# kai422/DAS3R

Hardware: AMD Instinct MI355X
Metric: render fwd+bwd Msplats/s at 1080p (higher is better)
Workload: dtype f32; 1 GPU; 1M random splats, 1920x1080, SH degree 3, forward+backward (BASELINE.json configs[3], constant P); splats_per_gpu=1000000, splats_per_gpu_final=1000000, init_steps=30, sh_degree=3, num_rendered=2614506, api=GaussianRasterizer.forward + autograd backward (drop-in surface), parallelism=1 independent scenes, one per GPU

## Files before the change

### das3r_amd/csrc/api.hip

```cpp
#include <stdarg.h>
#include <string.h>

#include <vector>

#include "common.h"
#include <algorithm>

namespace das3r {

static thread_local char g_err[512] = "";

void set_error(const char *fmt, ...) {
    va_list ap;
    va_start(ap, fmt);
    vsnprintf(g_err, sizeof(g_err), fmt, ap);
    va_end(ap);
}

struct ProfRec {
    const char *name;
    hipEvent_t start, stop;
};
static bool g_prof_on = false;
static std::vector<ProfRec> g_prof;
bool profile_enabled() { return g_prof_on; }
static std::vector<hipEvent_t> g_event_pool;
static hipEvent_t pooled_event() {
    if (!g_event_pool.empty()) { hipEvent_t e = g_event_pool.back(); g_event_pool.pop_back(); return e; }
    hipEvent_t e = nullptr;
    return hipEventCreate(&e) == hipSuccess ? e : nullptr;
}
void profile_begin(const char *name, hipStream_t s) {
    ProfRec r;
    r.name = name;
    r.start = pooled_event();
    r.stop = pooled_event();
    if (!r.start || !r.stop) return;
    (void)hipEventRecord(r.start, s);
    g_prof.push_back(r);
}
void profile_end(hipStream_t s) {
    if (!g_prof.empty()) (void)hipEventRecord(g_prof.back().stop, s);
}

static Switches g_sw;
static bool g_sw_loaded = false;
static int g_inject_fault = 0;
static int g_mutate = 0;
static void load_switches() {
    Switches w;
    memset(&w, 0, sizeof(w));
    auto env = [](const char *k) -> const char * { const char *e = getenv(k); return (e && e[0]) ? e : nullptr; };
    const char *e;
#ifdef DAS3R_EXPERIMENTS
    if ((e = env("DAS3R_SORT_IPL"))) { const int v = atoi(e); w.sort_ipl = (v == 4 || v == 8 || v == 16) ? v : 0; }
    w.sort_classic = (e = env("DAS3R_SORT")) && e[0] == 'c';
    w.no_sh_stage = getenv("DAS3R_NO_SH_STAGE") != nullptr;
    if ((e = env("DAS3R_ABLATE"))) { w.ablate_set = true; w.ablate = atoi(e); }
    if ((e = env("DAS3R_BWD_PAD_LDS"))) w.bwd_pad_lds = atoi(e);
    if ((e = env("DAS3R_FWD_PAD_LDS"))) w.fwd_pad_lds = atoi(e);
    if ((e = env("DAS3R_SCAN_ITEMS"))) { const int v = atoi(e); w.scan_items = (v == 1 || v == 2 || v == 4 || v == 8 || v == 16) ? v : 0; }
    w.fwd_no_prefetch = (e = env("DAS3R_FWD_PREFETCH")) && e[0] == '0';
#endif
    w.rect_upstream = (e = env("DAS3R_RECT")) && e[0] == 'u';
    w.verbose = env("DAS3R_VERBOSE") != nullptr;
    if ((e = env("DAS3R_BINNING"))) w.binning = e[0] == 'l' ? 1 : (e[0] == 'r' ? -1 : (e[0] == 's' ? (strchr(e, '3') ? 3 : 2) : 0));
    w.capacity_exact = (e = env("DAS3R_CAPACITY")) && e[0] == 'e';
    w.fused_emit_off = (e = env("DAS3R_FUSED_EMIT")) && e[0] == '0';
    if ((e = env("DAS3R_SPLIT_COLOUR"))) w.split_colour = e[0] == '0' ? -1 : (e[0] == '1' ? 1 : 0);
    w.tile_lpt_off = (e = env("DAS3R_TILE_LPT")) && e[0] == '0';
    if ((e = env("DAS3R_RENDER"))) w.render_fwd = e[0] == 'q' ? 1 : (e[0] == 'r' ? 2 : (e[0] == 'l' ? 3 : (e[0] == 's' ? 4 : (e[0] == 'f' ? 5 : 0))));
    if ((e = env("DAS3R_RENDER_BWD"))) {
        w.render_bwd = e[0] == 'd' ? 1 : (e[0] == 'm' ? 2 : (strncmp(e, "stream", 6) == 0 ? 5 : (e[0] == 's' ? 3 : (e[0] == 'b' ? 6 : (e[0] == 'f' ? 7 : 0)))));
        if (w.render_bwd == 6) {
            const char *d = e;
            while (*d && (*d < '0' || *d > '9')) d++;
            w.render_bwd_mb = *d ? atoi(d) : 128;
            const char *pp = strchr(e, 'p');
            w.render_bwd_pix = pp ? atoi(pp + 1) : 0;
            const char *po = strchr(e, 'o');
            w.render_bwd_occ = po ? atoi(po + 1) : 5;
        }
        if (w.render_bwd == 7) {
            const char *d = e;
            while (*d && (*d < '0' || *d > '9')) d++;
            w.render_bwd_mb = *d ? atoi(d) : 128;
            w.render_bwd_pix = strchr(e, 'q') ? 9 : (strchr(e, 's') ? 8 : 0);
        }
        if (w.render_bwd == 3) {
            const char *d = e;
            while (*d && (*d < '0' || *d > '9')) d++;
            w.render_bwd_mb = (*d ? atoi(d) : 256) + (strncmp(e, "scana", 5) == 0 ? 1000 : 0);
        }
    }
    if ((e = env("DAS3R_BWD_REDUCE"))) { w.bwd_reduce_set = true; w.bwd_reduce_shfl = e[0] == 's'; }
    w.tickets = -1;
    if ((e = env("DAS3R_TICKETS"))) w.tickets = e[0] == 'a' ? 0 : (e[0] == 'n' ? 1 << 30 : ((e[0] >= '1' && e[0] <= '9') ? atoi(e) : -1));
    w.deterministic = (e = env("DAS3R_DETERMINISTIC")) && e[0] != '0';
    w.bwd_buckets = -1;
    if ((e = env("DAS3R_BWD_BUCKETS"))) w.bwd_buckets = atoi(e);
    w.tile_strip = 8;
    w.tile_chunk = -1;
    if ((e = env("DAS3R_TILE_CHUNK"))) { const int v = atoi(e); w.tile_chunk = (v >= 0 && v <= 64 && (v & (v - 1)) == 0) ? v : -1; }
    if ((e = env("DAS3R_TILE_STRIP"))) w.tile_strip = std::max(0, std::min(63, atoi(e)));
    w.inject_fault = g_inject_fault;
    w.mutate = g_mutate;
    g_sw = w;
    __atomic_store_n(&g_sw_loaded, true, __ATOMIC_RELEASE);
}
const Switches &switches() {
    if (!__atomic_load_n(&g_sw_loaded, __ATOMIC_ACQUIRE)) load_switches();
    return g_sw;
}

constexpr int MAX_DEVICES = 64;
static int g_threads_on_device[MAX_DEVICES] = {};
struct ThreadRegistrar {
    bool on[MAX_DEVICES] = {};
    void add(int dev) {
        if (!on[dev]) { on[dev] = true; __atomic_fetch_add(&g_threads_on_device[dev], 1, __ATOMIC_RELAXED); }
    }
    ~ThreadRegistrar() {
// ... 31 lines not shown
    if (forced > 0) return true;
    return sh_degree >= 2 && P >= SPLIT_MIN_P && !no_backward;
}

struct SideStreams {
    struct Entry { int dev; hipStream_t caller; SideStream ss; };
    std::vector<Entry> all;
    ~SideStreams() {
        for (auto &e : all) {
            (void)hipEventDestroy(e.ss.fork);
            (void)hipEventDestroy(e.ss.join);
            (void)hipStreamDestroy(e.ss.stream);
        }
    }
};
static int side_stream_for(hipStream_t s, SideStream *out) {
    static thread_local SideStreams streams;
    int dev = 0;
    HIP_TRY(hipGetDevice(&dev));
    for (auto &e : streams.all)
        if (e.dev == dev && e.caller == s) { *out = e.ss; return DAS3R_OK; }
    SideStream ss = {nullptr, nullptr, nullptr, 0};
    int cus = 0;
    HIP_TRY(hipDeviceGetAttribute(&cus, hipDeviceAttributeMultiprocessorCount, dev));
    ss.colour_blocks = COLOUR_WGS_PER_CU * (cus > 0 ? cus : 1);
    HIP_TRY(hipStreamCreateWithFlags(&ss.stream, hipStreamNonBlocking));
    HIP_TRY(hipEventCreateWithFlags(&ss.fork, hipEventDisableTiming));
    HIP_TRY(hipEventCreateWithFlags(&ss.join, hipEventDisableTiming));
    streams.all.push_back(SideStreams::Entry{dev, s, ss});
    *out = ss;
    return DAS3R_OK;
}

int sort_ipl_override() { return switches().sort_ipl; }
#ifdef DAS3R_EXPERIMENTS
bool use_onesweep() { return !switches().sort_classic; }
#else
bool use_onesweep() { return true; }
#endif
bool use_tight_rect() { return !switches().rect_upstream; }

void compute_layout(int P, int64_t I, int W, int H, Layout *L, bool shjac) {
    memset(L, 0, sizeof(*L));
    const size_t Pn = P > 0 ? (size_t)P : 1, In = I > 0 ? (size_t)I : 1;
    L->capacity = I;
    L->tiles_x = (W + TILE_X - 1) / TILE_X;
    L->tiles_y = (H + TILE_Y - 1) / TILE_Y;
    L->ntiles = L->tiles_x * L->tiles_y;
    L->tbits = tile_bits(L->ntiles);
    L->tile_passes = (L->tbits + 7) / 8;
    L->dbits = 0;
    L->kbits = L->tbits;
    L->kshift = 0;
    L->part_passes = L->tile_passes;
    L->chunksP = sort_num_chunks(P);
    L->chunksI = sort_num_chunks(I);
    size_t o = 0;
    auto take = [&](size_t b) { size_t r = o; o += align_up(b); return r; };
    L->g_keyA = take(4 * Pn);
    L->g_keyB = take(4 * Pn);
    L->g_valA = take(4 * Pn);
    L->g_valB = take(4 * Pn);
    L->pub.sorted_idx = L->g_valA;
    L->pub.depth_key = L->g_keyA;
    L->pub.xy = take(16 * SPLAT_REC * Pn);
    L->pub.conic_opacity = L->pub.xy + 16;
    L->pub.rgbd = L->pub.xy + 32;
    L->pub.splat_stride = 16 * SPLAT_REC;
    L->pub.clamped = take(Pn);
    L->pub.tiles_touched = take(4 * Pn);
    L->pub.offsets = take(4 * Pn);
    L->g_hist = take(4 * (size_t)RADIX_SIZE * (size_t)(L->chunksP > 0 ? L->chunksP : 1));
    L->g_totals = take(4 * RADIX_SIZE);
    L->g_blocksums = take(4 * (size_t)div_up((int64_t)Pn, 4096));
    L->g_count = take(256);
    L->g_off_by_gid = take(4 * Pn);
    L->g_rect = take(4 * Pn);
    L->g_dhist = take(4 * 256);
    L->g_ghist = take(4 * 4 * RADIX_SIZE);
    L->g_ticket = take(256);
    L->g_status = take(onesweep_status_bytes((int64_t)Pn, 4));
    L->g_scan_status = take(scan_status_bytes((int)Pn));
    L->g_ctrl_bytes = o - L->g_ghist;
    if (shjac) L->g_shjac = take(4 * 9 * Pn);
    L->pub.geom_bytes = o;
    o = 0;
    L->b_keyA = take(4 * In);
    L->b_keyB = take(4 * In);
    L->b_valA = take(4 * In);
    L->b_valB = take(4 * In);
    L->b_hist = take(4 * (size_t)RADIX_SIZE * (size_t)(L->chunksI > 0 ? L->chunksI : 1));
    L->b_totals = take(4 * RADIX_SIZE);
    L->b_gid_of = take(4 * In);
    L->b_slot = take(4 * In);
    L->b_e2 = take(4 * In);
    L->b_ghist = take(4 * 4 * RADIX_SIZE);
    L->b_ticket = take(256);
    L->b_status = take(onesweep_status_bytes((int64_t)In, L->tile_passes + 1));
    L->b_ctrl_bytes = o - L->b_ghist;
    L->b_ckpt = take(((size_t)In / BUCKET + (size_t)(L->ntiles > 0 ? L->ntiles : 1) + 2) * 256 * 16);
    L->pub.binning_bytes = o;
    const size_t npix_d = (size_t)W * (size_t)H;
    L->d_ckpt = take(((size_t)In / BUCKET + (size_t)(L->ntiles > 0 ? L->ntiles : 1) + 2) * 256 * 16);
    L->d_recs = take(16 * SPLAT_REC * Pn);
    L->d_dpix = take(4 * 3 * (npix_d > 0 ? npix_d : 1));
    L->d_bg = take(16);
// ... 245 lines not shown
    Mailbox *mb = &T->mb;
    auto check_slot = [&](uint32_t i, bool wait) -> int {
        if (!T->pending[i]) return DAS3R_OK;
        const int r = examine_check_slot(mb->host + CHECK_WORD0 + 2 * i, T->pending[i], wait, s);
        if (r == 1) return DAS3R_OK;
        T->pending[i] = 0;
        return r;
    };
    for (uint32_t i = 0; i < CHECK_SLOTS; i++)
        if ((rc = check_slot(i, false))) return rc;
    uint32_t late_tag = 0;
    unsigned long long *&arrive_ring = T->arrive_ring;
    constexpr uint32_t ARRIVE_SLOTS = 16, ARRIVE_WORDS = 8 + 64 * 8;
    if (!arrive_ring) {
        HIP_TRY(hipMalloc((void **)&arrive_ring, ARRIVE_SLOTS * ARRIVE_WORDS * sizeof(unsigned long long)));
        HIP_TRY(hipMemsetAsync(arrive_ring, 0, ARRIVE_SLOTS * ARRIVE_WORDS * sizeof(unsigned long long), s));
        HIP_TRY(hipStreamSynchronize(s));
    }
    Verdict &verdict = T->verdict;
    constexpr int64_t LOCAL_AVG = 384;
    const uint32_t too_long = mb->host[10];
    if (too_long) mb->host[10] = 0;
    const uint32_t want_bits = mb->host[11];
    if (want_bits) mb->host[11] = 0;
    if (verdict.P != P || verdict.W != W || verdict.H != H) {
        const uint32_t gen = verdict.gen + 1u ? verdict.gen + 1u : 1u;
        verdict = Verdict{P, W, H, -1, 0, 0, 64, gen};
        if (T->pending_valid) {
            verdict.fine = T->pending_fine;
            verdict.forwards = T->pending_forwards;
            T->pending_valid = false;
        }
    }
    const bool decide_fine = (verdict.forwards++ & 511u) == 0u;
    auto next_gen = [&]() { verdict.gen = verdict.gen + 1u ? verdict.gen + 1u : 1u; };
    if (verdict.last_I < 0) {
    } else if (too_long == verdict.gen && !(verdict.last_seg && verdict.seg_extra == 0 && L.tile_passes < 3 && seg_dbits(L, L.tile_passes + 1) > 0)) {
        if (verdict.clean >= 256u) verdict.backoff = 64;
        verdict.radix_left = verdict.backoff;
        if (verdict.backoff < 4096) verdict.backoff *= 2;
        verdict.clean = 0;
        next_gen();
    } else if (too_long == verdict.gen || want_bits == verdict.gen) {
        verdict.seg_extra = 1;
        next_gen();
    }
    const int forced = switches().binning;
    bool local = use_onesweep() && (forced == 1 || (forced == 0 && verdict.radix_left == 0 && verdict.last_I <= LOCAL_AVG * L.ntiles));
    constexpr int64_t SEG_AVG = 384;
    const int seg_passes = L.tile_passes + ((forced == 3 || (forced == 0 && verdict.seg_extra)) ? 1 : 0);
    const int seg_bits = (use_onesweep() && seg_passes <= 3) ? seg_dbits(L, seg_passes) : 0;
    bool seg = !local && seg_bits > 0 && (forced >= 2 || (forced == 0 && verdict.radix_left == 0 && verdict.last_I >= 0 &&
                                                           (verdict.last_I >> std::min(seg_bits, 20)) <= SEG_AVG * L.ntiles));
    const uint32_t *seg_dhist = nullptr;
    auto apply_seg = [&]() {
        L.dhist_ptr = seg_dhist;
        if (seg) {
            L.dbits = seg_bits;
            L.kbits = L.tbits + seg_bits;
            L.kshift = std::min(16, 32 - L.kbits);
            L.part_passes = seg_passes;
        }
    };
    verdict.last_seg = seg;
    if (local || seg) verdict.clean++;
    if (forced == 0 && verdict.radix_left > 0) verdict.radix_left--;
    const uint32_t count_tag = ++mb->seq ? mb->seq : ++mb->seq;
    unsigned long long *arrive = arrive_ring + (size_t)(count_tag % ARRIVE_SLOTS) * ARRIVE_WORDS;
    struct Join {
        hipStream_t s;
        const das3r_raster_args *a;
        const das3r_raster_in *in;
        char *const *geom;
        const Layout *L;
        SideStream side;
        bool forked, pending;
        int launch() {
            if (!forked) return DAS3R_OK;
            forked = false;
            pending = true;
            return launch_sh_colour(a, in, *geom, *L, &side);
        }
        int now() {
            const int r = launch();
            if (r) return r;
            if (!pending) return DAS3R_OK;
            pending = false;
            HIP_TRY(hipStreamWaitEvent(s, side.join, 0));
            return DAS3R_OK;
        }
        ~Join() {
            if (pending) (void)hipStreamWaitEvent(s, side.join, 0);
        }
    } join = {s, a, in, &saved->geom, &L, {nullptr, nullptr, nullptr, 0}, false, false};
    auto split_side = [&](int binning_path, const SideStream **side) -> int {
        *side = nullptr;
        if (!split_colour_rule(in->shs != nullptr, a->sh_degree, P, binning_path, no_backward, switches().split_colour)) return DAS3R_OK;
        const int r = side_stream_for(s, &join.side);
        if (r) return r;
        *side = &join.side;
        return DAS3R_OK;
    };
    auto bin_and_render = [&](int64_t cap, bool local_order, bool ctrl_zeroed, uint32_t *count_out = nullptr, uint32_t count_out_tag = 0,
                              uint32_t *emit_slot = nullptr ) -> int {
        int r;
        const bool fused_scan = use_onesweep();
        const bool seg = L.dbits > 0;
        if (!emit_slot) {
            if (fused_scan) {
                if ((r = launch_binning_scan_emit(P, cap, out->radii, saved->geom, saved->binning, L, ctrl_zeroed, count_out, count_out_tag, a->debug != 0,
                                                  s, local_order || seg))) return r;
            } else if ((r = launch_scan(P, saved->geom, L, nullptr, 0, a->debug != 0, s))) return r;
        }
        uint32_t *host_late = nullptr;
        if (cap > 0) {
            late_tag = ++mb->seq ? mb->seq : ++mb->seq;
            const uint32_t slot = late_tag % CHECK_SLOTS;
            if ((r = check_slot(slot, true))) return r;
            T->pending[slot] = late_tag;
            host_late = mb->dev + CHECK_WORD0 + 2 * slot;
            saved->check_word = (void *)(mb->host + CHECK_WORD0 + 2 * slot);
            saved->check_tag = late_tag;
        }
        uint32_t *dead_keys = nullptr;
        if ((r = launch_binning(P, cap, W, H, out->radii, saved->geom, saved->binning, saved->img, L, fused_scan, host_late, late_tag,
                                a->debug != 0, s, &dead_keys, emit_slot, mb->dev + 10, verdict.gen))) return r;
        if ((r = join.launch())) return r;
        LocalBin lb = {(float4 *)(saved->binning + L.b_ckpt), nullptr, nullptr, nullptr, nullptr, verdict.gen, (uint32_t)(P - 1), (uint32_t)cap};
        if (decide_fine && cap > 0 && use_quad_lanes(L, lb)) {
            const uint32_t tag = ++mb->seq ? mb->seq : ++mb->seq;
            if ((r = launch_list_skew(saved->img, saved->binning, saved->geom, L, (uint32_t)cap, (uint32_t)(P - 1), mb->dev + 13, tag, a->debug != 0, s))) return r;
            if ((r = mailbox_wait(mb, 14, tag, s))) return r;
            const int64_t longest = (int64_t)mb->host[13], mean = (verdict.last_I > 0 ? verdict.last_I : cap) / std::max(L.ntiles, 1);
            verdict.longest = (uint32_t)longest;
            const uint32_t crowd16 = mb->host[15];
            verdict.fine = (longest > mean + (mean * 4) / 5 && longest >= 4096) || crowd16 >= CROWDED16;
            if (switches().verbose) fprintf(stderr, "[das3r] tile lists: longest %lld, mean %lld, %.1f of 64 consecutive entries in one quadrant -> %s kernels\n", (long long)longest,
                                            (long long)mean, crowd16 / 16.0, verdict.fine ? "2x2-region" : "block");
        }
        lb.prefer_regions = verdict.fine;
        lb.tile_order = nullptr;
        if (verdict.fine && cap > 0 && use_quad_lanes(L, lb) && L.ntiles <= 1024 && !switches().tile_lpt_off && (switches().render_fwd == 0 || switches().render_fwd == 5)) {
            if ((r = launch_tile_lpt(saved->img, L, (uint32_t)cap, a->debug != 0, s))) return r;
            lb.tile_order = (const uint32_t *)(saved->img + L.i_order);
        }
        if (verdict.fine && cap > 0 && use_quad_lanes(L, lb)) {
            const uint32_t hint = std::min<uint32_t>(63u, verdict.longest / (uint32_t)BUCKET + 2u);
            saved->flags |= 1u | (hint << 8);
        }
        if (local_order && cap > 0) {
            lb.point_list = (uint32_t *)(saved->binning + L.pub.point_list);
            lb.slot_list = (uint32_t *)(saved->binning + L.b_slot);
            lb.keys = dead_keys;
            lb.host_flag = mb->dev + 10;
        }
        if ((r = join.now())) return r;
        return launch_render_forward(a, in->colors_precomp, out->out_color, saved->geom, saved->binning, saved->img, L, lb, s, out->out_invdepth,
                                     depth ? (float4 *)(saved->binning + L.d_ckpt) : nullptr);
    };
    auto prefiltered_ok = [&]() -> int {
        if (!a->prefiltered || mb->host[12] != count_tag) return DAS3R_OK;
        set_error("Point is filtered although prefiltered is set. This shouldn't happen!");
        return DAS3R_ERR_INVALID_ARG;
    };
    int64_t I, cap;
    if ((local || seg) && verdict.last_I >= 0 && a->capacity_hint != -1 && !switches().capacity_exact) {
        cap = std::max(verdict.last_I + verdict.last_I / 4, verdict.peak_I + verdict.peak_I / 20) + 4096;
        if (cap > (int64_t)0x7FFFFF00) cap = (int64_t)0x7FFFFF00;
        compute_layout(P, cap, W, H, &L, shjac);
        apply_seg();
        saved->binning = alloc_binning(user, depth ? L.d_bytes : L.pub.binning_bytes);
        if (!saved->binning) { set_error("scratch allocation failed (binning %zu B)", L.pub.binning_bytes); return DAS3R_ERR_ALLOC; }
        char *&emit_ring = T->emit_ring;
        bool &emit_ring_dirty = T->emit_ring_dirty;
        uint32_t &emit_last_tag = T->emit_last_tag;
        constexpr size_t EMIT_SLOT_BYTES = sizeof(uint32_t) * EMIT_SLOT_WORDS + sizeof(unsigned long long) * EMIT_STATUS_GRANULES;
        const bool fused_emit = local && grid_is_resident(div_up(P, 256)) && !switches().fused_emit_off;
        uint32_t *emit_slot = nullptr;
        if (fused_emit) {
            if (!emit_ring) {
                HIP_TRY(hipMalloc((void **)&emit_ring, ARRIVE_SLOTS * EMIT_SLOT_BYTES));
                emit_ring_dirty = true;
            }
            if (emit_ring_dirty || count_tag < emit_last_tag) {
                HIP_TRY(hipMemsetAsync(emit_ring, 0, ARRIVE_SLOTS * EMIT_SLOT_BYTES, s));
                emit_ring_dirty = false;
            }
            emit_last_tag = count_tag;
            emit_slot = (uint32_t *)(emit_ring + (size_t)(count_tag % ARRIVE_SLOTS) * EMIT_SLOT_BYTES);
            const EmitArgs em = {(unsigned long long *)(emit_slot + EMIT_SLOT_WORDS), count_tag, emit_slot + 64, emit_slot,
                                 (uint32_t *)(saved->binning + L.b_keyA), (uint32_t *)(saved->binning + L.b_gid_of),
                                 (uint32_t *)(saved->geom + L.g_off_by_gid), (uint32_t)cap, L.tbits, (uint32_t *)(saved->geom + L.g_count), mb->dev};
            emit_ring_dirty = true;
            if ((rc = launch_preprocess(a, in, out->radii, saved->geom, saved->img, saved->binning + L.b_ghist, L.b_ctrl_bytes, L, nullptr, mb->dev,
                                        count_tag, s, &em, nullptr, nullptr, aa))) return rc;
            if ((rc = bin_and_render(cap, true, true, nullptr, 0, emit_slot))) return rc;
            emit_ring_dirty = false;
        } else {
            uint32_t *dhist = nullptr, *dhist_next = nullptr;
            if (seg && !dhist_slots(s, &dhist, &dhist_next)) {
                dhist = (uint32_t *)(saved->geom + L.g_dhist);
                HIP_TRY(hipMemsetAsync(dhist, 0, 4 * 256, s));
            }
            seg_dhist = dhist;
            apply_seg();
            const SideStream *side = nullptr;
            if ((rc = split_side(1, &side))) return rc;
            if ((rc = launch_preprocess(a, in, out->radii, saved->geom, saved->img, saved->binning + L.b_ghist, L.b_ctrl_bytes, L, nullptr, mb->dev,
                                        count_tag, s, nullptr, dhist, dhist_next, aa, side))) return rc;
            join.forked = side != nullptr;
            if ((rc = bin_and_render(cap, local, true, mb->dev, count_tag))) return rc;
        }
        if ((rc = mailbox_wait(mb, 2, count_tag, s))) return rc;
        if ((rc = prefiltered_ok())) return rc;
        I = (int64_t)mb->host[0];
        if (I > (int64_t)0x7FFFFF00) { set_error("num_rendered %lld exceeds 2^31", (long long)I); return DAS3R_ERR_OVERFLOW; }
        verdict.last_I = I;
        verdict.peak_I = std::max(I, verdict.peak_I - verdict.peak_I / 1024);
        if (I > cap) {
            cap = I;
            compute_layout(P, cap, W, H, &L, shjac);
            saved->binning = alloc_binning(user, depth ? L.d_bytes : L.pub.binning_bytes);
            if (!saved->binning) { set_error("scratch allocation failed (binning %zu B)", L.pub.binning_bytes); return DAS3R_ERR_ALLOC; }
            apply_seg();
            HIP_TRY(hipMemsetAsync(saved->geom + L.g_ghist, 0, L.g_ctrl_bytes, s));
            HIP_TRY(hipMemsetAsync(saved->img + L.pub.ranges, 0, 8 * (size_t)L.ntiles, s));
            if ((rc = bin_and_render(cap, local, false))) return rc;
        }
    } else {
        uint32_t *dhist = nullptr, *dhist_next = nullptr;
        if (seg && !dhist_slots(s, &dhist, &dhist_next)) {
            dhist = (uint32_t *)(saved->geom + L.g_dhist);
            HIP_TRY(hipMemsetAsync(dhist, 0, 4 * 256, s));
        }
        seg_dhist = dhist;
        const SideStream *side = nullptr;
        if ((rc = split_side((local || seg) ? 1 : 0, &side))) return rc;
        if ((rc = launch_preprocess(a, in, out->radii, saved->geom, saved->img, nullptr, 0, L, arrive, mb->dev, count_tag, s, nullptr, dhist, dhist_next, aa, side))) return rc;
        join.forked = side != nullptr;
        if (!local && !seg && (rc = launch_depth_sort(P, saved->geom, L, 0, nullptr, 0, a->debug != 0, s))) return rc;
        if ((rc = mailbox_wait(mb, 2, count_tag, s))) return rc;
        if ((rc = prefiltered_ok())) return rc;
        I = cap = (int64_t)mb->host[0];
        if (cap > (int64_t)0x7FFFFF00) { set_error("num_rendered %lld exceeds 2^31", (long long)cap); return DAS3R_ERR_OVERFLOW; }
        verdict.last_I = I;
        verdict.peak_I = std::max(I, verdict.peak_I - verdict.peak_I / 1024);
        if (local && forced == 0 && I > LOCAL_AVG * L.ntiles) {
            local = false;
            if ((rc = join.now())) return rc;
            if ((rc = launch_depth_sort(P, saved->geom, L, 0, nullptr, 0, a->debug != 0, s))) return rc;
        }
        compute_layout(P, cap, W, H, &L, shjac);
        apply_seg();
        saved->binning = alloc_binning(user, depth ? L.d_bytes : L.pub.binning_bytes);
        if (!saved->binning) { set_error("scratch allocation failed (binning %zu B)", L.pub.binning_bytes); return DAS3R_ERR_ALLOC; }
        if (!local && !seg && (rc = launch_depth_sort(P, saved->geom, L, 1, saved->binning + L.b_ghist, L.b_ctrl_bytes, a->debug != 0, s))) return rc;
        if ((rc = bin_and_render(cap, local, !local && !seg))) return rc;
    }
    if (a->debug && late_tag && (rc = check_slot(late_tag % CHECK_SLOTS, true))) return rc;
    saved->num_rendered = I;
    saved->capacity = cap;
    if (depth) saved->flags |= DEPTH_SAVED_FLAG;
    if (shjac) saved->flags |= SHJAC_SAVED_FLAG;
    return I;
}

static bool shjac_saved(const das3r_raster_args *a, const das3r_raster_in *in, const das3r_raster_saved *saved) {
    return (saved->flags & SHJAC_SAVED_FLAG) != 0 && in->shs != nullptr && a->sh_degree >= 2;
}

extern "C" int das3r_raster_backward(const das3r_raster_args *a, const das3r_raster_in *in, const das3r_raster_saved *saved,
                                     const float *dL_dpix, const das3r_raster_grads *g, das3r_stream_t stream) {
    hipStream_t s = (hipStream_t)stream;
    int rc = validate(a, in);
    if (rc) return rc;
    const int P = a->P;
    if (P == 0) return DAS3R_OK;
    const bool chained = g && g->chain;
    if (!saved || !saved->geom || !saved->img || !dL_dpix || !g || !g->dL_dmeans2D || (!chained && (!g->dL_dopacities || !g->dL_dmeans3D)) ||
        (saved && saved->num_rendered > 0 && !g->scratch)) {
        set_error("das3r_raster_backward: null saved state / gradient buffer");
        return DAS3R_ERR_INVALID_ARG;
    }
    const bool has_sh = in->shs != nullptr, has_cov = in->cov3D_precomp != nullptr;
// ... 280 lines not shown
```

### das3r_amd/csrc/common.h

```cpp
#pragma once
#include <hip/hip_runtime.h>
#include <stdint.h>
#include <stdio.h>

#include "../../include/das3r_raster.h"
#include "pretransform_math.h"

#define TILE_X 16
#define TILE_Y 16
#define TILE_PIX 256
#define WAVE 64
#define NEAR_PLANE 0.001f

namespace das3r {

void set_error(const char *fmt, ...);

struct Switches {
    int sort_ipl;
    bool sort_classic;
    bool rect_upstream;
    bool verbose;
    int binning;
    bool capacity_exact;
    bool fused_emit_off;
    bool no_sh_stage;
    int render_fwd;
    int render_bwd;
    int render_bwd_mb;
    int tile_chunk;
    int scan_items;
    bool deterministic;
    int render_bwd_occ;
    bool tile_lpt_off;
    int render_bwd_pix;
    bool bwd_reduce_set, bwd_reduce_shfl;
    bool ablate_set;
    int ablate;
    int tickets;
    int bwd_pad_lds, fwd_pad_lds;
    int bwd_buckets;
    int inject_fault;
    int mutate;
    bool fwd_no_prefetch;
    int split_colour;
    int tile_strip;
};
const Switches &switches();

#define HIP_TRY(expr)                                                                          \
    do {                                                                                       \
        hipError_t _e = (expr);                                                                \
        if (_e != hipSuccess) {                                                                \
            das3r::set_error("%s failed: %s (%s:%d)", #expr, hipGetErrorString(_e), __FILE__, __LINE__); \
            return DAS3R_ERR_HIP;                                                              \
        }                                                                                      \
    } while (0)

#define KERNEL_CHECK(stream, debug, name)                                                      \
    do {                                                                                       \
        hipError_t _e = hipGetLastError();                                                     \
        if (_e == hipSuccess && (debug)) _e = hipStreamSynchronize(stream);                    \
        if (_e != hipSuccess) {                                                                \
            das3r::set_error("kernel %s failed: %s", name, hipGetErrorString(_e));             \
            return DAS3R_ERR_HIP;                                                              \
        }                                                                                      \
    } while (0)

bool profile_enabled();
void profile_begin(const char *name, hipStream_t s);
void profile_end(hipStream_t s);
struct ProfTimer {
    hipStream_t s;
    bool on;
    ProfTimer(const char *name, hipStream_t stream) : s(stream), on(profile_enabled()) {
        if (on) profile_begin(name, s);
    }
    ~ProfTimer() {
        if (on) profile_end(s);
    }
};

unsigned long long *pair_counters();
constexpr int PHASE_WORDS = 16, PHASE_COPIES = 64;
#ifdef DAS3R_EXPERIMENTS
#define PHASE_BEGIN()                                                                      \
    __shared__ unsigned long long phase_w_[8];                                             \
    unsigned long long phase_t_ = 0ull;                                                    \
    if (pairs != nullptr && threadIdx.x == 0) {                                            \
        for (int k_ = 0; k_ < 8; k_++) phase_w_[k_] = 0ull;                                \
        phase_t_ = clock64();                                                              \
    }
#define PHASE_MARK(k)                                                                      \
    if (pairs != nullptr && threadIdx.x == 0) {                                            \
        const unsigned long long now_ = clock64();                                         \
        phase_w_[(k) & 7] += now_ - phase_t_;                                              \
        phase_t_ = now_;                                                                   \
    }
// ... 30 lines not shown
#define WG_STAMP(k)
#define SCAN_STAMP(k)
#define BLK_STAMP(ptr, r, k)
#endif

#define DAS3R_LAUNCH(kernel, grid, block, shmem, stream, ...)                \
    do {                                                                     \
        das3r::ProfTimer _pt(#kernel, stream);                               \
        hipLaunchKernelGGL(kernel, grid, block, shmem, stream, __VA_ARGS__); \
    } while (0)

static inline size_t align_up(size_t x, size_t a = 256) { return (x + a - 1) / a * a; }
static inline int div_up(int64_t a, int64_t b) { return (int)((a + b - 1) / b); }

constexpr int RADIX_BITS = 8;
constexpr int RADIX_SIZE = 1 << RADIX_BITS;
constexpr int SORT_WAVES_PER_BLOCK = 4;
int sort_ipl_override();
static inline int sort_items_per_lane(int64_t n) {
    const int o = sort_ipl_override();
    return o ? o : (n >= (int64_t)(1 << 21) ? 16 : (n >= (1 << 17) ? 8 : 4));
}
static inline int sort_num_chunks(int64_t n) { return n == 0 ? 0 : div_up(n, (int64_t)WAVE * sort_items_per_lane(n)); }
__host__ __device__ static inline int tile_digit_width(int tbits) {
    const int passes = (tbits + 7) / 8;
    return passes > 0 ? (tbits + passes - 1) / passes : 8;
}
static inline int tile_bits(int ntiles) {
    int b = 0;
    while ((1 << b) < ntiles) b++;
    return b < 1 ? 1 : b;
}

constexpr int BUCKET = 1024;
constexpr int SPLAT_REC = 4;

constexpr uint32_t DEPTH_SAVED_FLAG = 2u;
constexpr uint32_t SHJAC_SAVED_FLAG = 4u;
constexpr uint32_t NO_BACKWARD_IN_FLAG = 8u;
constexpr uint32_t ANTIALIAS_FLAG = 16u;
struct Layout {
    das3r_raster_layout pub;
    size_t g_keyA, g_keyB, g_valA, g_valB, g_hist, g_totals, g_blocksums, g_count, g_off_by_gid, g_rect;
    size_t b_keyA, b_keyB, b_valA, b_valB, b_hist, b_totals, b_gid_of, b_slot;
    size_t b_e2;
    size_t b_ckpt;
    size_t d_ckpt, d_recs, d_dpix, d_bg, d_dz, d_bytes;
    size_t g_ghist, g_ticket, g_status, g_scan_status, g_ctrl_bytes;
    int64_t capacity;
    size_t b_ghist, b_ticket, b_status, b_ctrl_bytes;
    int tiles_x, tiles_y, ntiles, tbits, tile_passes;
    int chunksP, chunksI;
    int dbits, kbits, kshift;
    int part_passes;
    size_t g_dhist;
    size_t g_shjac;
    const uint32_t *dhist_ptr;
    size_t i_order;
};
static inline int seg_dbits(const Layout &L, int passes) { return 8 * (passes < 3 ? passes : 3) - L.tbits; }

struct LocalBin {
    float4 *ckpt;
    uint32_t *point_list, *slot_list;
    uint32_t *keys;
    uint32_t *host_flag;
    uint32_t flag_value;
    uint32_t last_g, cap;
    bool prefer_regions;
    const uint32_t *tile_order;
};
void compute_layout(int P, int64_t I, int W, int H, Layout *L, bool shjac = false);

struct EmitArgs {
    unsigned long long *status;
    uint32_t tag;
    uint32_t *ghist;
    uint32_t *err;
    uint32_t *tile_keys, *gids, *off_by_gid;
    uint32_t cap;
    int tbits;
    uint32_t *count;
    uint32_t *count_out;
};
constexpr int EMIT_SLOT_WORDS = 64 + 4 * 256;
constexpr int EMIT_STATUS_GRANULES = 1024;

constexpr int COLOUR_WGS_PER_CU = 4;
struct SideStream {
    hipStream_t stream;
    hipEvent_t fork, join;
    int colour_blocks;
};
int launch_preprocess(const das3r_raster_args *a, const das3r_raster_in *in, int32_t *radii, char *geom, char *img, char *binning_ctrl,
                      size_t binning_ctrl_bytes, const Layout &L, unsigned long long *arrive, uint32_t *host_out, uint32_t tag,
                      hipStream_t s, const EmitArgs *emit, uint32_t *dhist, uint32_t *dhist_next, bool aa ,
                      const SideStream *side = nullptr);
int launch_sh_colour(const das3r_raster_args *a, const das3r_raster_in *in, char *geom, const Layout &L, const SideStream *side);
int launch_mark_visible(int P, const float *means3D, const float *viewmatrix, uint8_t *present, hipStream_t s);
int launch_depth_sort(int P, char *geom, const Layout &L, int part, char *binning_ctrl, size_t binning_ctrl_bytes, bool debug, hipStream_t s);
int launch_scan(int P, char *geom, const Layout &L, uint32_t *host_out, uint32_t tag, bool debug, hipStream_t s, bool index_order = false);
int launch_scan_emit(int P, int64_t cap, const int32_t *radii, char *geom, char *binning, const Layout &L, uint32_t *host_out, uint32_t tag,
                     bool debug, hipStream_t s, bool index_order = false);
size_t scan_status_bytes(int P);
int launch_binning_scan_emit(int P, int64_t I, const int32_t *radii, char *geom, char *binning, const Layout &L, bool ctrl_zeroed,
                             uint32_t *host_out, uint32_t tag, bool debug, hipStream_t s, bool index_order = false);
size_t onesweep_status_bytes(int64_t n, int passes);
int launch_onesweep_depth_sort(int P, char *geom, const Layout &L, int part, uint32_t *zero_ptr, uint32_t zero_words, bool debug,
                               hipStream_t s);
int launch_onesweep_partition(int64_t cap, char *geom, char *binning, const Layout &L, uint32_t **keys_final, bool debug, hipStream_t s,
                              uint32_t *ghist_override = nullptr, uint32_t *err_override = nullptr);
bool use_row_private(int64_t instances, int ntiles);
bool use_quad_lanes(const Layout &L, const LocalBin &lb);
inline PreXform pre_xform(const das3r_raster_in *in) {
    PreXform x = {nullptr, nullptr, nullptr, nullptr, nullptr, nullptr, nullptr, nullptr, nullptr};
    if (in && in->pre) {
        const das3r_pretransform *p = in->pre;
        x = PreXform{p->xyz, p->rot, p->scaling, p->opacity_raw, p->conf_flat, p->mask_index, p->R, p->t, p->Lq};
    }
    return x;
}
int launch_render_forward_regions(const das3r_raster_args *a, float *out_color, char *geom, char *binning, char *img, const Layout &L, const LocalBin &lb,
                                  hipStream_t s, float *out_invdepth, float4 *dckpt);
// ... 80 lines not shown
```

### das3r_amd/csrc/render_common.h

```cpp
#pragma once
#include "common.h"

namespace das3r {

struct StagedSplat {
    float4 xyh;
    float4 co;
    float4 rgbd;
};

__device__ __forceinline__ float4 lds_read4(const float4 *p) {
    const float4 v = *p;
    asm volatile("" ::"v"(v.w));
    return v;
}

__device__ __forceinline__ StagedSplat null_splat() {
    StagedSplat z;
    z.xyh = make_float4(0.f, 0.f, -1e30f, -1e30f);
    z.co = make_float4(0.f, 0.f, 0.f, 0.f);
    z.rgbd = make_float4(0.f, 0.f, 0.f, 0.f);
    return z;
}

// ... 182 lines not shown
        for (int lk = 1; lk <= G; lk++) {
#pragma unroll
            for (int i = 0; i < E; i++)
                if (!(i & (1 << (lk - 1)))) ce64(v[i], v[i ^ ((1 << lk) - 1)]);
#pragma unroll
            for (int lj = lk - 2; lj >= 0; lj--)
#pragma unroll
                for (int i = 0; i < E; i++)
                    if (!((i >> lj) & 1)) ce64(v[i], v[i | (1 << lj)]);
        }
#pragma unroll
        for (int m = 0; m < E; m++) key[lane * E + m] = v[m];
    }
    __builtin_amdgcn_fence(__ATOMIC_ACQ_REL, "wavefront");
    for (int lk = G + 1; lk <= LOGN; lk++) {
        {
            const int sh = lk - G;
            const int block = lane >> sh, hbase = lane & ((1 << sh) - 1);
            const int lo0 = (block << lk) + hbase, hi0 = (block << lk) + ((1 << lk) - 1) - hbase;
            double a[H], b[H];
#pragma unroll
            for (int m = 0; m < H; m++) {
                a[m] = key[lo0 + (m << sh)];
                b[m] = key[hi0 - (m << sh)];
            }
#pragma unroll
            for (int m = 0; m < H; m++) ce64(a[m], b[m]);
#pragma unroll
            for (int t = G - 2; t >= 0; t--)
#pragma unroll
                for (int m = 0; m < H; m++)
                    if (!((m >> t) & 1)) {
                        ce64(a[m], a[m | (1 << t)]);
                        ce64(b[m | (1 << t)], b[m]);
                    }
#pragma unroll
            for (int m = 0; m < H; m++) {
                key[lo0 + (m << sh)] = a[m];
                key[hi0 - (m << sh)] = b[m];
            }
        }
        __builtin_amdgcn_fence(__ATOMIC_ACQ_REL, "wavefront");
        for (int R = lk - G; R > 0;) {
            const int g = R < G ? R : G;
            if (g == 1) butterfly_group<1, E>(key, lane, R);
            else if (g == 2) butterfly_group<2, E>(key, lane, R);
            else if (g == 3) butterfly_group<3, E>(key, lane, R);
            __builtin_amdgcn_fence(__ATOMIC_ACQ_REL, "wavefront");
            R -= g;
        }
    }
}

struct NoMark {
    __device__ __forceinline__ void operator()(int) const {}
};
template <bool DEPTH = false, class Mark = NoMark>
__device__ __forceinline__ bool local_order_tile(const LocalBin &lb, const uint2 range, const float4 *__restrict__ xyh,
                                                 const float4 *__restrict__ conic_opacity, const float4 *__restrict__ rgbd,
                                                 StagedSplat *stage , uint32_t *s_gid , const int tid,
                                                 const Mark mark = Mark()) {
    const int n = (int)(range.y - range.x);
    uint32_t *pl = lb.point_list + range.x, *sl = lb.slot_list + range.x;
    if (n <= TILE_PIX) {
        unsigned long long *s_key = reinterpret_cast<unsigned long long *>(s_gid);
        unsigned long long key = 0;
        uint32_t g = 0, slot = 0;
        float4 r0 = make_float4(0.f, 0.f, 0.f, 0.f), r1 = r0, r2 = r0;
        if (tid < n) {
            g = min(pl[tid], lb.last_g);
            slot = sl[tid];
            r0 = xyh[(size_t)g * SPLAT_REC];
            r1 = conic_opacity[(size_t)g * SPLAT_REC];
            r2 = rgbd[(size_t)g * SPLAT_REC];
            key = ((unsigned long long)__float_as_uint(r2.w) << 32) | (unsigned long long)g;
        }
        if (tid < ((n + 7) & ~7)) s_key[tid] = tid < n ? key : ~0ull;
        __syncthreads();
        if (tid < n) {
            int rank = 0;
            for (int j = 0; j < n; j += 8) {
                unsigned long long o[8];
#pragma unroll
                for (int u = 0; u < 8; u++) o[u] = s_key[j + u];
#pragma unroll
                for (int u = 0; u < 8; u++) rank += o[u] < key ? 1 : 0;
            }
            stage[rank].xyh = r0;
            stage[rank].co = r1;
            if constexpr (DEPTH) stage[rank].rgbd = staged_invz(r2);
            else stage[rank].rgbd = r2;
            pl[rank] = g;
            sl[rank] = slot;
        } else {
            stage[tid] = null_splat();
        }
        return true;
    }
    if (n <= LOCAL_MAX) {
        unsigned long long *s_key = reinterpret_cast<unsigned long long *>(stage);
        uint32_t *s_slot = reinterpret_cast<uint32_t *>(stage) + 2 * LOCAL_MAX;
        const int N = n <= 2 * TILE_PIX ? 2 * TILE_PIX : LOCAL_MAX;
        for (int i = tid; i < N; i += TILE_PIX) {
            unsigned long long k = SORT_PAD;
            if (i < n) {
                const uint32_t g = min(pl[i], lb.last_g);
                s_gid[i] = g;
                s_slot[i] = sl[i];
                k = ((unsigned long long)__float_as_uint(rgbd[(size_t)g * SPLAT_REC].w) << 32) | (unsigned long long)i;
            }
            s_key[i] = k;
        }
        __syncthreads();
        mark(6);
        if (N == 2 * TILE_PIX) {
            if (tid < 64) wave_bitonic_sort<3>(reinterpret_cast<double *>(stage), tid);
// ... 156 lines not shown
```

### das3r_amd/csrc/sort.hip

```cpp
#include "granule.h"
#include "segkey.h"
#include <algorithm>
#include "splat_math.h"

namespace das3r {

template <int IPL>
__global__ void __launch_bounds__(256) radix_hist_kernel(const uint32_t *__restrict__ keys, uint32_t cap, const uint32_t *__restrict__ n_ptr,
                                                         int shift, uint32_t mask, int nchunks, uint32_t *__restrict__ hist) {
    const uint32_t n = n_ptr ? min(*n_ptr, cap) : cap;
    __shared__ uint32_t cnt[SORT_WAVES_PER_BLOCK][RADIX_SIZE];
    const int lane = __lane_id(), wave = threadIdx.x >> 6;
    const int chunk = blockIdx.x * SORT_WAVES_PER_BLOCK + wave;
    const uint32_t base = (uint32_t)chunk * 64u * (uint32_t)IPL;
    uint32_t k[IPL];
#pragma unroll
    for (int s = 0; s < IPL; s++) {
        const uint32_t i = base + s * 64 + lane;
        k[s] = (chunk < nchunks && i < n) ? keys[i] : 0u;
    }
#pragma unroll
    for (int d = lane; d < RADIX_SIZE; d += 64) cnt[wave][d] = 0;
    __builtin_amdgcn_wave_barrier();
    if (chunk >= nchunks) return;
// ... 228 lines not shown
    uint32_t *hist = (uint32_t *)(geom + L.g_hist), *totals = (uint32_t *)(geom + L.g_totals);
    if (P == 0) return DAS3R_OK;
    int rc;
    if (use_onesweep()) return launch_onesweep_depth_sort(P, geom, L, part, (uint32_t *)binning_ctrl, (uint32_t)(binning_ctrl_bytes / 4), debug, s);
#ifdef DAS3R_EXPERIMENTS
    if (part == 1) return DAS3R_OK;
    if ((rc = radix_pass(keyA, nullptr, keyB, valB, P, 0, 8, hist, totals, debug, s))) return rc;
    if ((rc = radix_pass(keyB, valB, keyA, valA, P, 8, 8, hist, totals, debug, s))) return rc;
    if ((rc = radix_pass(keyA, valA, keyB, valB, P, 16, 8, hist, totals, debug, s))) return rc;
    if ((rc = radix_pass(keyB, valB, nullptr, valA, P, 24, 8, hist, totals, debug, s))) return rc;
#else
    (void)keyA; (void)keyB; (void)valA; (void)valB; (void)hist; (void)totals; (void)rc;
#endif
    return DAS3R_OK;
}

int launch_binning_scan_emit(int P, int64_t I, const int32_t *radii, char *geom, char *binning, const Layout &L, bool ctrl_zeroed,
                             uint32_t *host_out, uint32_t tag, bool debug, hipStream_t s, bool index_order) {
    if (I == 0 || P == 0) return DAS3R_OK;
    if (!ctrl_zeroed) HIP_TRY(hipMemsetAsync(binning + L.b_ghist, 0, L.b_ctrl_bytes, s));
    return launch_scan_emit(P, I, radii, geom, binning, L, host_out, tag, debug, s, index_order);
}

int launch_binning(int P, int64_t I, int W, int H, const int32_t *radii, char *geom, char *binning, char *img, const Layout &L,
                   bool fused_scan, uint32_t *host_late, uint32_t tag, bool debug, hipStream_t s, uint32_t **dead_keys, uint32_t *emit_slot,
                   uint32_t *seg_host_flag, uint32_t seg_flag_value) {
    const uint32_t *n_ptr = (const uint32_t *)(geom + L.g_count);
    (void)W; (void)H;
    uint2 *ranges = (uint2 *)(img + L.pub.ranges);
    if (I == 0 || P == 0) return DAS3R_OK;
    uint32_t *keyA = (uint32_t *)(binning + L.b_keyA), *keyB = (uint32_t *)(binning + L.b_keyB);
    uint32_t *valA = (uint32_t *)(binning + L.b_valA), *valB = (uint32_t *)(binning + L.b_valB);
    uint32_t *hist = (uint32_t *)(binning + L.b_hist), *totals = (uint32_t *)(binning + L.b_totals);
    uint32_t *gid_of = (uint32_t *)(binning + L.b_gid_of), *inv = (uint32_t *)(binning + L.b_slot);
    const bool onesweep = use_onesweep();
    (void)onesweep;
#ifdef DAS3R_EXPERIMENTS
    if (!fused_scan) {
    const int emit_blocks = div_up(P, 256) < 1024 ? div_up(P, 256) : 1024;
    DAS3R_LAUNCH(emit_kernel, dim3(emit_blocks), dim3(256), 0, s, P, L.tiles_x, L.tiles_y,
                 (const uint32_t *)(geom + L.pub.sorted_idx), (const uint32_t *)(geom + L.pub.tiles_touched),
                 (const uint32_t *)(geom + L.pub.offsets), (const float4 *)(geom + L.pub.xy), radii, keyA, gid_of, (uint32_t)I,
                 onesweep ? (uint32_t *)(binning + L.b_ghist) : (uint32_t *)nullptr, L.tbits, use_tight_rect() ? 1 : 0);
    KERNEL_CHECK(s, debug, "emit");
    }
#else
    (void)radii; (void)fused_scan; (void)gid_of;
#endif
    if (onesweep) {
        uint32_t *kfinal = nullptr;
        int rc1 = launch_onesweep_partition(I, geom, binning, L, &kfinal, debug, s, emit_slot ? emit_slot + 64 : nullptr, emit_slot);
        if (rc1) return rc1;
        if (dead_keys) *dead_keys = kfinal;
        if (L.dbits > 0) {
            uint32_t *other = kfinal == keyA ? keyB : keyA;
            return launch_segment_sort(I, n_ptr, kfinal, L.kshift, (uint32_t *)(binning + L.pub.point_list), (uint32_t *)(binning + L.b_slot),
                                       (const uint32_t *)(geom + L.pub.depth_key), (uint32_t)(P - 1), other, seg_host_flag, seg_flag_value, debug, s,
                                       L.dbits, ranges, (const uint32_t *)(geom + L.g_ticket) + 8, host_late, tag, (uint32_t)switches().inject_fault);
        }
        const int rearm = emit_slot ? EMIT_SLOT_WORDS : 0;
        DAS3R_LAUNCH(tile_ranges_kernel, dim3(div_up(std::max<int64_t>(div_up(I, 4), rearm), 256)), dim3(256), 0, s, (uint32_t)I, n_ptr, kfinal, ranges,
                     emit_slot ? emit_slot : (uint32_t *)(geom + L.g_ticket) + 8, host_late, tag, (uint32_t)rearm, (uint32_t)switches().inject_fault, L.dbits + L.kshift);
        KERNEL_CHECK(s, debug, "tile_ranges");
        return DAS3R_OK;
    }
#ifdef DAS3R_EXPERIMENTS
    uint32_t *kin = keyA, *vin = nullptr, *kout = keyB, *vout = valB;
    int shift = 0, rc;
    for (int p = 0; p < L.tile_passes; p++) {
        const int dw = tile_digit_width(L.tbits), bits = (L.tbits - shift) < dw ? (L.tbits - shift) : dw;
        const bool last = p == L.tile_passes - 1;
        if ((rc = radix_pass(kin, vin, kout, vout, I, shift, bits, hist, totals, debug, s, last ? gid_of : nullptr, last ? inv : nullptr, n_ptr)))
            return rc;
        shift += bits;
        uint32_t *t = kin; kin = kout; kout = t;
        vin = vout;
        vout = (vout == valB) ? valA : valB;
    }
    if (dead_keys) *dead_keys = kin;
    DAS3R_LAUNCH(tile_ranges_kernel, dim3(div_up(div_up(I, 4), 256)), dim3(256), 0, s, (uint32_t)I, n_ptr, kin, ranges,
                 (uint32_t *)(geom + L.g_ticket) + 8, host_late, tag, 0u, (uint32_t)switches().inject_fault, 0);
    KERNEL_CHECK(s, debug, "tile_ranges");
#else
    (void)keyA; (void)keyB; (void)valA; (void)valB; (void)hist; (void)totals; (void)inv;
#endif
    return DAS3R_OK;
}

}
```

Before: 1161 Msplats/s.

## Use coarse depth buckets from radix keys to speed local per-tile ordering

When per-tile local depth ordering is chosen, the binning keys now carry some depth bits beside the tile id. The render forward uses the top bucket bits (up to 32 buckets) to rank each splat by comparing only against others in its bucket, instead of against all splats in the tile. It falls back to the full ranking when a bucket exceeds 128 entries, and it is disabled when the fused emit path is used. This adds a depth histogram pass and key-layout changes, and a layout flag now separates segmented sorting from depth-bucketed keys.

Result: faster. 1181 Msplats/s (median of 5 runs) (+1.7%).

```diff
diff --git a/das3r_amd/csrc/api.hip b/das3r_amd/csrc/api.hip
--- a/das3r_amd/csrc/api.hip
+++ b/das3r_amd/csrc/api.hip
@@ -68,6 +68,7 @@
     w.capacity_exact = (e = env("DAS3R_CAPACITY")) && e[0] == 'e';
     w.fused_emit_off = (e = env("DAS3R_FUSED_EMIT")) && e[0] == '0';
     if ((e = env("DAS3R_SPLIT_COLOUR"))) w.split_colour = e[0] == '0' ? -1 : (e[0] == '1' ? 1 : 0);
+    if ((e = env("DAS3R_LOCAL_BUCKETS"))) w.local_buckets = e[0] == '0' ? -1 : (e[0] == '1' ? 1 : 0);
     w.tile_lpt_off = (e = env("DAS3R_TILE_LPT")) && e[0] == '0';
     if ((e = env("DAS3R_RENDER"))) w.render_fwd = e[0] == 'q' ? 1 : (e[0] == 'r' ? 2 : (e[0] == 'l' ? 3 : (e[0] == 's' ? 4 : (e[0] == 'f' ? 5 : 0))));
     if ((e = env("DAS3R_RENDER_BWD"))) {
@@ -205,6 +206,7 @@
     L->dbits = 0;
     L->kbits = L->tbits;
     L->kshift = 0;
+    L->segmented = false;
     L->part_passes = L->tile_passes;
     L->chunksP = sort_num_chunks(P);
     L->chunksI = sort_num_chunks(I);
@@ -556,14 +558,18 @@
     const int seg_bits = (use_onesweep() && seg_passes <= 3) ? seg_dbits(L, seg_passes) : 0;
     bool seg = !local && seg_bits > 0 && (forced >= 2 || (forced == 0 && verdict.radix_left == 0 && verdict.last_I >= 0 &&
                                                            (verdict.last_I >> std::min(seg_bits, 20)) <= SEG_AVG * L.ntiles));
+    const int lbuck_bits = use_onesweep() ? std::min(seg_dbits(L, L.tile_passes), 16) : 0;
+    bool lbuck = local && lbuck_bits > 0 && switches().local_buckets >= 0;
     const uint32_t *seg_dhist = nullptr;
     auto apply_seg = [&]() {
         L.dhist_ptr = seg_dhist;
-        if (seg) {
-            L.dbits = seg_bits;
-            L.kbits = L.tbits + seg_bits;
+        if (seg || (local && lbuck)) {
+            const int bits = seg ? seg_bits : lbuck_bits;
+            L.dbits = bits;
+            L.kbits = L.tbits + bits;
             L.kshift = std::min(16, 32 - L.kbits);
-            L.part_passes = seg_passes;
+            L.segmented = seg;
+            if (seg) L.part_passes = seg_passes;
         }
     };
     verdict.last_seg = seg;
@@ -609,7 +615,7 @@
                               uint32_t *emit_slot = nullptr ) -> int {
         int r;
         const bool fused_scan = use_onesweep();
-        const bool seg = L.dbits > 0;
+        const bool seg = L.segmented;
         if (!emit_slot) {
             if (fused_scan) {
                 if ((r = launch_binning_scan_emit(P, cap, out->radii, saved->geom, saved->binning, L, ctrl_zeroed, count_out, count_out_tag, a->debug != 0,
@@ -657,6 +663,10 @@
             lb.slot_list = (uint32_t *)(saved->binning + L.b_slot);
             lb.keys = dead_keys;
             lb.host_flag = mb->dev + 10;
+            if (L.dbits > 0 && !L.segmented && !emit_slot) {
+                lb.dbits = L.dbits;
+                lb.kshift = L.kshift;
+            }
         }
         if ((r = join.now())) return r;
         return launch_render_forward(a, in->colors_precomp, out->out_color, saved->geom, saved->binning, saved->img, L, lb, s, out->out_invdepth,
@@ -671,6 +681,8 @@
     if ((local || seg) && verdict.last_I >= 0 && a->capacity_hint != -1 && !switches().capacity_exact) {
         cap = std::max(verdict.last_I + verdict.last_I / 4, verdict.peak_I + verdict.peak_I / 20) + 4096;
         if (cap > (int64_t)0x7FFFFF00) cap = (int64_t)0x7FFFFF00;
+        const bool fused_emit = local && grid_is_resident(div_up(P, 256)) && !switches().fused_emit_off;
+        if (fused_emit) lbuck = false;
         compute_layout(P, cap, W, H, &L, shjac);
         apply_seg();
         saved->binning = alloc_binning(user, depth ? L.d_bytes : L.pub.binning_bytes);
@@ -679,7 +691,6 @@
         bool &emit_ring_dirty = T->emit_ring_dirty;
         uint32_t &emit_last_tag = T->emit_last_tag;
         constexpr size_t EMIT_SLOT_BYTES = sizeof(uint32_t) * EMIT_SLOT_WORDS + sizeof(unsigned long long) * EMIT_STATUS_GRANULES;
-        const bool fused_emit = local && grid_is_resident(div_up(P, 256)) && !switches().fused_emit_off;
         uint32_t *emit_slot = nullptr;
         if (fused_emit) {
             if (!emit_ring) {
@@ -702,7 +713,7 @@
             emit_ring_dirty = false;
         } else {
             uint32_t *dhist = nullptr, *dhist_next = nullptr;
-            if (seg && !dhist_slots(s, &dhist, &dhist_next)) {
+            if ((seg || (local && lbuck)) && !dhist_slots(s, &dhist, &dhist_next)) {
                 dhist = (uint32_t *)(saved->geom + L.g_dhist);
                 HIP_TRY(hipMemsetAsync(dhist, 0, 4 * 256, s));
             }
@@ -733,7 +744,7 @@
         }
     } else {
         uint32_t *dhist = nullptr, *dhist_next = nullptr;
-        if (seg && !dhist_slots(s, &dhist, &dhist_next)) {
+        if ((seg || (local && lbuck)) && !dhist_slots(s, &dhist, &dhist_next)) {
             dhist = (uint32_t *)(saved->geom + L.g_dhist);
             HIP_TRY(hipMemsetAsync(dhist, 0, 4 * 256, s));
         }
diff --git a/das3r_amd/csrc/common.h b/das3r_amd/csrc/common.h
--- a/das3r_amd/csrc/common.h
+++ b/das3r_amd/csrc/common.h
@@ -44,6 +44,7 @@
     int mutate;
     bool fwd_no_prefetch;
     int split_colour;
+    int local_buckets;
     int tile_strip;
 };
 const Switches &switches();
@@ -180,6 +181,7 @@
     int tiles_x, tiles_y, ntiles, tbits, tile_passes;
     int chunksP, chunksI;
     int dbits, kbits, kshift;
+    bool segmented;
     int part_passes;
     size_t g_dhist;
     size_t g_shjac;
@@ -197,6 +199,7 @@
     uint32_t last_g, cap;
     bool prefer_regions;
     const uint32_t *tile_order;
+    int dbits, kshift;
 };
 void compute_layout(int P, int64_t I, int W, int H, Layout *L, bool shjac = false);
 
diff --git a/das3r_amd/csrc/render_common.h b/das3r_amd/csrc/render_common.h
--- a/das3r_amd/csrc/render_common.h
+++ b/das3r_amd/csrc/render_common.h
@@ -258,6 +258,106 @@
     }
 }
 
+constexpr int RANK_MAX = 128;
+template <bool DEPTH, int E>
+__device__ __forceinline__ int local_order_buckets(const LocalBin &lb, const uint2 range, const float4 *__restrict__ xyh,
+                                                   const float4 *__restrict__ conic_opacity, const float4 *__restrict__ rgbd,
+                                                   StagedSplat *stage, uint32_t *s_gid, const int tid) {
+    const int n = (int)(range.y - range.x);
+    uint32_t *pl = lb.point_list + range.x, *sl = lb.slot_list + range.x;
+    const uint32_t *kw = lb.keys + range.x;
+    unsigned long long *s_key = E == 1 ? reinterpret_cast<unsigned long long *>(s_gid) : reinterpret_cast<unsigned long long *>(stage);
+    uint32_t *s_cnt = E == 1 ? s_gid + 2 * TILE_PIX : reinterpret_cast<uint32_t *>(stage) + 2 * LOCAL_MAX;
+    const int bsh = lb.kshift + (lb.dbits > 5 ? lb.dbits - 5 : 0);
+    const uint32_t bmask = (1u << (lb.dbits > 5 ? 5 : lb.dbits)) - 1u;
+    if (tid < 32) s_cnt[tid] = 0u;
+    uint32_t g[E], slot[E], b[E];
+#pragma unroll
+    for (int u = 0; u < E; u++) {
+        const int i = u * TILE_PIX + tid;
+        g[u] = 0u; slot[u] = 0u; b[u] = 0u;
+        if (i < n) {
+            g[u] = min(pl[i], lb.last_g);
+            slot[u] = sl[i];
+            b[u] = (kw[i] >> bsh) & bmask;
+        }
+    }
+    float4 r0 = make_float4(0.f, 0.f, 0.f, 0.f), r1 = r0, r2 = r0;
+    unsigned long long key[E];
+#pragma unroll
+    for (int u = 0; u < E; u++) {
+        const int i = u * TILE_PIX + tid;
+        key[u] = ~0ull;
+        if (i < n) {
+            if constexpr (E == 1) {
+                r0 = xyh[(size_t)g[u] * SPLAT_REC];
+                r1 = conic_opacity[(size_t)g[u] * SPLAT_REC];
+                r2 = rgbd[(size_t)g[u] * SPLAT_REC];
+                key[u] = ((unsigned long long)__float_as_uint(r2.w) << 32) | (unsigned long long)i;
+            } else {
+                key[u] = ((unsigned long long)__float_as_uint(rgbd[(size_t)g[u] * SPLAT_REC].w) << 32) | (unsigned long long)i;
+            }
+        }
+    }
+    __syncthreads();
+#pragma unroll
+    for (int u = 0; u < E; u++) {
+        const int i = u * TILE_PIX + tid;
+        const uint32_t mine = i < n ? b[u] : ~0u, before = __shfl_up(mine, 1);
+        const uint64_t heads = __ballot((tid & 63) == 0 || before != mine);
+        const uint64_t above = (tid & 63) == 63 ? 0ull : heads >> ((tid & 63) + 1);
+        const int run = above ? __ffsll((unsigned long long)above) : 64 - (tid & 63);
+        if (i < n && ((heads >> (tid & 63)) & 1ull)) atomicAdd(&s_cnt[b[u]], (uint32_t)run);
+        if (i < ((n + 7) & ~7)) s_key[i] = key[u];
+    }
+    __syncthreads();
+    const int lane = tid & 63;
+    const uint32_t c = s_cnt[lane & 31];
+    uint32_t incl = c, most = c;
+#pragma unroll
+    for (int d = 1; d < 32; d <<= 1) {
+        const uint32_t up = __shfl_up(incl, d, 32);
+        if ((lane & 31) >= d) incl += up;
+        most = max(most, (uint32_t)__shfl_xor(most, d, 32));
+    }
+    if (__builtin_amdgcn_readfirstlane(most) > (uint32_t)RANK_MAX) {
+        __syncthreads();
+        return -1;
+    }
+#pragma unroll
+    for (int u = 0; u < E; u++) {
+        const int i = u * TILE_PIX + tid;
+        const uint32_t end = __shfl(incl, (int)b[u], 32), cnt = __shfl(c, (int)b[u], 32);
+        if (i < n) {
+            const int lo = (int)(end - cnt) & ~7, hi = (int)end;
+            int at = lo;
+            for (int j = lo; j < hi; j += 8) {
+                unsigned long long o[8];
+#pragma unroll
+                for (int q = 0; q < 8; q++) o[q] = s_key[j + q];
+#pragma unroll
+                for (int q = 0; q < 8; q++) at += o[q] < key[u] ? 1 : 0;
+            }
+            at = min(at, n - 1);
+            if constexpr (E == 1) {
+                stage[at].xyh = r0;
+                stage[at].co = r1;
+                if constexpr (DEPTH) stage[at].rgbd = staged_invz(r2);
+                else stage[at].rgbd = r2;
+            } else {
+                s_gid[at] = g[u];
+            }
+            pl[at] = g[u];
+            sl[at] = slot[u];
+        } else if (E == 1) {
+            stage[tid] = null_splat();
+        }
+    }
+    if constexpr (E == 1) return 1;
+    __syncthreads();
+    return 0;
+}
+
 struct NoMark {
     __device__ __forceinline__ void operator()(int) const {}
 };
@@ -268,6 +368,15 @@
                                                  const Mark mark = Mark()) {
     const int n = (int)(range.y - range.x);
     uint32_t *pl = lb.point_list + range.x, *sl = lb.slot_list + range.x;
+    if (lb.dbits > 0 && n <= LOCAL_MAX) {
+        const int r = n <= TILE_PIX       ? local_order_buckets<DEPTH, 1>(lb, range, xyh, conic_opacity, rgbd, stage, s_gid, tid)
+                      : n <= 2 * TILE_PIX ? local_order_buckets<DEPTH, 2>(lb, range, xyh, conic_opacity, rgbd, stage, s_gid, tid)
+                                          : local_order_buckets<DEPTH, 4>(lb, range, xyh, conic_opacity, rgbd, stage, s_gid, tid);
+        if (r >= 0) {
+            mark(7);
+            return r != 0;
+        }
+    }
     if (n <= TILE_PIX) {
         unsigned long long *s_key = reinterpret_cast<unsigned long long *>(s_gid);
         unsigned long long key = 0;
diff --git a/das3r_amd/csrc/sort.hip b/das3r_amd/csrc/sort.hip
--- a/das3r_amd/csrc/sort.hip
+++ b/das3r_amd/csrc/sort.hip
@@ -304,7 +304,7 @@
         int rc1 = launch_onesweep_partition(I, geom, binning, L, &kfinal, debug, s, emit_slot ? emit_slot + 64 : nullptr, emit_slot);
         if (rc1) return rc1;
         if (dead_keys) *dead_keys = kfinal;
-        if (L.dbits > 0) {
+        if (L.segmented) {
             uint32_t *other = kfinal == keyA ? keyB : keyA;
             return launch_segment_sort(I, n_ptr, kfinal, L.kshift, (uint32_t *)(binning + L.pub.point_list), (uint32_t *)(binning + L.b_slot),
                                        (const uint32_t *)(geom + L.pub.depth_key), (uint32_t)(P - 1), other, seg_host_flag, seg_flag_value, debug, s,
```
